# cxy1997/3D_adapt_auto_driving

Measured on AMD Instinct MI355X. Metric: KITTI scenes/s end-to-end eval_rcnn (joint RPN+RCNN, synthetic 16384-pt scenes), higher is better.
Workload: dtype f32; 1 GPU; BASELINE.json configs[2]: full PointRCNN RPN+RCNN inference, default.yaml shapes, random-init weights, batch=8 synthetic KITTI scenes x 16384 pts per GPU per step; scene=synth.scenes (SURVEY 8d: uniform clutter + ground + 10 dense cars), parallelism=scene-sharded x1, one final all_gather of detections, detections_gathered=652455, batch_slots=14, look_ahead=12, steps_per_launch=2

## Files before the change

### 3d_adapt_auto_driving_amd/csrc/mfma_stream.hpp

```cpp
#pragma once

#define RT_VM_DRAIN __builtin_amdgcn_s_waitcnt(0x0F70);
#define RT_LOAD_W(dst, rs, krow)                                                                          \
    _Pragma("unroll") for (int s = 0; s < 64; ++s)                                                        \
        dst[s] = __uint_as_float(__builtin_amdgcn_raw_buffer_load_b32(rs, lane_off, (unsigned int)((krow) + s) * 512u, 0)); \
    __builtin_amdgcn_sched_barrier(0);
#define RT_STAGE_HOOK_LO(T, wf, wn, RS, krow, FIRST, HOOK, LOFF)                                                     \
    {                                                                                                     \
        f32x4 a0 = *reinterpret_cast<const f32x4 *>((T) + j * RT_LD + 64 * h);                            \
        f32x4 a1 = *reinterpret_cast<const f32x4 *>((T) + (32 + j) * RT_LD + 64 * h);                     \
        _Pragma("unroll") for (int g = 0; g < 16; ++g) {                                                  \
            f32x4 n0 = a0, n1 = a1;                                                                       \
            if (g < 15) {                                                                                 \
                n0 = *reinterpret_cast<const f32x4 *>((T) + j * RT_LD + 64 * h + 4 * (g + 1));            \
                n1 = *reinterpret_cast<const f32x4 *>((T) + (32 + j) * RT_LD + 64 * h + 4 * (g + 1));     \
            }                                                                                             \
            __builtin_amdgcn_sched_barrier(0);                                                            \
            if ((FIRST) && g == 0) {                                                                      \
                const f32x16 zero = {0};                                                                  \
                acc0 = __builtin_amdgcn_mfma_f32_32x32x2f32(a0.x, wf[0], zero, 0, 0, 0);                  \
                acc1 = __builtin_amdgcn_mfma_f32_32x32x2f32(a1.x, wf[0], zero, 0, 0, 0);                  \
            } else {                                                                                      \
                acc0 = __builtin_amdgcn_mfma_f32_32x32x2f32(a0.x, wf[4 * g + 0], acc0, 0, 0, 0);          \
                acc1 = __builtin_amdgcn_mfma_f32_32x32x2f32(a1.x, wf[4 * g + 0], acc1, 0, 0, 0);          \
            }                                                                                             \
            _Pragma("unroll") for (int q = 0; q < 4; ++q)                                                 \
                wn[4 * g + q] = __uint_as_float(__builtin_amdgcn_raw_buffer_load_b32(                     \
                    RS, (LOFF), (unsigned int)((krow) + 4 * g + q) * 512u, 0));                           \
            __builtin_amdgcn_sched_barrier(0);                                                            \
            HOOK(g)                                                                                       \
            acc0 = __builtin_amdgcn_mfma_f32_32x32x2f32(a0.y, wf[4 * g + 1], acc0, 0, 0, 0);              \
            acc1 = __builtin_amdgcn_mfma_f32_32x32x2f32(a1.y, wf[4 * g + 1], acc1, 0, 0, 0);              \
            acc0 = __builtin_amdgcn_mfma_f32_32x32x2f32(a0.z, wf[4 * g + 2], acc0, 0, 0, 0);              \
            acc1 = __builtin_amdgcn_mfma_f32_32x32x2f32(a1.z, wf[4 * g + 2], acc1, 0, 0, 0);              \
            acc0 = __builtin_amdgcn_mfma_f32_32x32x2f32(a0.w, wf[4 * g + 3], acc0, 0, 0, 0);              \
            acc1 = __builtin_amdgcn_mfma_f32_32x32x2f32(a1.w, wf[4 * g + 3], acc1, 0, 0, 0);              \
            a0 = n0; a1 = n1;                                                                             \
        }                                                                                                 \
    }
#define RT_STAGE_HOOK(T, wf, wn, RS, krow, FIRST, HOOK) RT_STAGE_HOOK_LO(T, wf, wn, RS, krow, FIRST, HOOK, lane_off)
#define RT_NO_HOOK(g)
#define RT_STAGE(T, wf, wn, RS, krow, FIRST) RT_STAGE_HOOK(T, wf, wn, RS, krow, FIRST, RT_NO_HOOK)
#define RT_EPILOGUE(T, bias, RELU)                                                                        \
    {                                                                                                     \
        const float bcol = (bias);                                                                        \
        _Pragma("unroll") for (int r = 0; r < 16; ++r) {                                                  \
            const int row = (r & 3) + 8 * (r >> 2) + 4 * h;                                               \
            const float v0 = acc0[r] + bcol, v1 = acc1[r] + bcol;                                         \
            (T)[row * RT_LD + 32 * w + j] = (RELU) ? fmaxf(v0, 0.f) : v0;                                 \
            (T)[(32 + row) * RT_LD + 32 * w + j] = (RELU) ? fmaxf(v1, 0.f) : v1;                          \
        }                                                                                                 \
    }
```

### 3d_adapt_auto_driving_amd/csrc/rpn_tail.hip

```cpp
#include <hip/hip_runtime.h>

#include "common.hpp"
#include "mfma_stream.hpp"
#include "../../include/prcnn_hip.h"

namespace prcnn {

typedef float f32x16 __attribute__((ext_vector_type(16)));
typedef float f32x4 __attribute__((ext_vector_type(4)));

constexpr int RT_ROWS = 64;
constexpr int RT_LD = 128 + 4;
#ifndef RT_IROWS
#define RT_IROWS 4
#endif

struct RpnTailArgs {
    long rows;
    int n, m;
    const float *known;
    const int *idx;
    const float *weight;
    const float *wcat;
    const float *bcat;
    const float *wc2, *bc2;
    float *feats, *cls, *reg;
    int n_reg;
    unsigned int *ticket;
    int xcd_split;
    const float *xyz;
    float *boxes;
    float loc_scope, loc_bin_size, anchor[3];
};

__device__ __forceinline__ float fmod_two_pi(float a)
{
    constexpr double B0 = (double)(float)(2.0 * M_PI), B1 = B0 * 1099511627776.0 , B2 = B1 * 1099511627776.0;
    constexpr double I0 = 1.0 / B0, I1 = 1.0 / B1, I2 = 1.0 / B2;
    double r = __builtin_fabs((double)a);
    r = __builtin_fma(-__builtin_trunc(r * I2), B2, r);
    r = __builtin_fma(-__builtin_trunc(r * I1), B1, r);
    r = __builtin_fma(-__builtin_trunc(r * I0), B0, r);
    r = r < 0.0 ? r + B0 : r;
    r = r < 0.0 ? r + B0 : r;
    r = r >= B0 ? r - B0 : r;
    r = r >= B0 ? r - B0 : r;
    return __builtin_copysignf((float)r, a);
}

__global__ __launch_bounds__(256, 1) void rpn_tail_kernel(const RpnTailArgs a)
{
    __shared__ float T0[RT_ROWS * RT_LD];
    __shared__ float T1[RT_ROWS * RT_LD];
    __shared__ float X0[RT_ROWS * RT_LD];
    __shared__ float X1[RT_ROWS * RT_LD];
    __shared__ unsigned int slot[2];
    const int tid = threadIdx.x, lane = tid & 63, j = lane & 31, h = lane >> 5;
    const int w = __builtin_amdgcn_readfirstlane(tid >> 6);
    const int chunk = tid & 31, r0 = tid >> 5;
    const long tiles = (a.rows + RT_ROWS - 1) / RT_ROWS;
    const unsigned int lane_off = ((unsigned int)(64 * h) * 128u + (unsigned int)(32 * w + j)) * 4u;
    const __amdgpu_buffer_rsrc_t rs = __builtin_amdgcn_make_buffer_rsrc((void *)a.wcat, 0, 768 * 128 * 4, 0x00020000);
    const float wd0 = a.wc2[j], wd1 = a.wc2[j + 32], wd2 = a.wc2[j + 64], wd3 = a.wc2[j + 96], bd = a.bc2[0];
    const f32x4 *known4 = reinterpret_cast<const f32x4 *>(a.known);
    const float bias1 = a.bcat[32 * w + j], bias2 = a.bcat[128 + 32 * w + j], biasc = a.bcat[256 + 32 * w + j],
                biasr1 = a.bcat[384 + 32 * w + j], biasr2 = a.bcat[512 + 32 * w + j];

    int nx_i, nx_cloud;
    float nx_w;
#define RT_FETCH_IDX(tt)                                                                                  \
    {                                                                                                     \
        long ge = (tt) * RT_ROWS + 16 * w + lane / 3;                                                     \
        if (ge >= a.rows) ge = a.rows - 1;  \
        const long el = ge * 3 + lane % 3;                                                                \
        nx_i = lane < 48 ? a.idx[el] : 0;                                                                 \
        nx_w = lane < 48 ? a.weight[el] : 0.f;                                                            \
        nx_cloud = (int)(ge / a.n);                                                                       \
    }
    f32x4 f[RT_IROWS][3];
#define RT_INTERP_ISSUE(rr)                                                                               \
    _Pragma("unroll") for (int q = 0; q < RT_IROWS; ++q) {                                                \
        const long cloud = __builtin_amdgcn_readlane(nx_cloud, 3 * ((rr) + q));                           \
        _Pragma("unroll") for (int e = 0; e < 3; ++e) {                                                   \
            const int i = __builtin_amdgcn_readlane(nx_i, 3 * ((rr) + q) + e);                            \
            f[q][e] = known4[(cloud * a.m + i) * 64 + lane];                                              \
        }                                                                                                 \
    }
#define RT_INTERP_ROW(rr, q)                                                                              \
    {                                                                                                     \
        const float w0 = __builtin_bit_cast(float, __builtin_amdgcn_readlane(__builtin_bit_cast(int, nx_w), 3 * ((rr) + (q)))); \
        const float w1 = __builtin_bit_cast(float, __builtin_amdgcn_readlane(__builtin_bit_cast(int, nx_w), 3 * ((rr) + (q)) + 1)); \
        const float w2 = __builtin_bit_cast(float, __builtin_amdgcn_readlane(__builtin_bit_cast(int, nx_w), 3 * ((rr) + (q)) + 2)); \
        const f32x4 v = (w0 * f[q][0] + w1 * f[q][1]) + w2 * f[q][2];                                     \
        float *dst = (lane < 32 ? X0 : X1) + (16 * w + (rr) + (q)) * RT_LD + 4 * (lane & 31);             \
        *reinterpret_cast<f32x4 *>(dst) = v;                                                              \
    }
#define RT_SIDE(rr, g)                                                                                    \
    if ((g) == 2) { RT_INTERP_ISSUE(rr) }                                                                 \
    else if ((g) >= 10 && (g) < 10 + RT_IROWS) { RT_INTERP_ROW(rr, (g) - 10) }
#define RT_SIDE0(g) RT_SIDE(0, g)
#define RT_SIDE1(g) RT_SIDE(RT_IROWS, g)
#define RT_SIDE2(g) RT_SIDE(2 * RT_IROWS, g)
#define RT_SIDE3(g) RT_SIDE(3 * RT_IROWS, g)
    f32x4 co[4];
#define RT_ROWS_OUT(g, TT, T, dst, ld, live)                                                              \
    if ((g) == 1 || (g) == 4) {                                                                       \
        _Pragma("unroll") for (int i = 0; i < 4; ++i) co[i] = *reinterpret_cast<const f32x4 *>((T) + (r0 + 8 * (i + ((g) == 4 ? 4 : 0))) * RT_LD + 4 * chunk); \
    } else if ((g) == 3 || (g) == 6) {                                                                \
        _Pragma("unroll") for (int i = 0; i < 4; ++i) {                                               \
            const unsigned int gr = (unsigned int)(TT) * RT_ROWS + r0 + 8 * (i + ((g) == 6 ? 4 : 0)); \
            if ((live) && gr < (unsigned int)a.rows) *reinterpret_cast<f32x4 *>((dst) + (gr * (unsigned int)(ld) + 4u * chunk)) = co[i]; \
        }                                                                                             \
    }
    static_assert(RT_IROWS == 4, "four stages carry four rounds of four rows");

    if (tid == 0) { slot[0] = atomicAdd(a.ticket, 1u); }
    __syncthreads();
    long t = __builtin_amdgcn_readfirstlane((int)slot[0]);
    float wa[64], wb[64];
    f32x16 acc0, acc1;
    RT_LOAD_W(wa, rs, 0)
    if (t < tiles) {
        RT_FETCH_IDX(t)
#pragma unroll
        for (int rr = 0; rr < 16; rr += RT_IROWS) {
            RT_INTERP_ISSUE(rr)
#pragma unroll
            for (int q = 0; q < RT_IROWS; ++q) RT_INTERP_ROW(rr, q)
        }
    }
    long tp = 0;
    bool last = false;
    for (unsigned int served = 0; t < tiles; ++served) {
        if (tid == 0) slot[(served + 1) & 1] = atomicAdd(a.ticket, 1u);
        RT_VM_DRAIN
        lds_barrier();
#define RT_REG_OUT(g) RT_ROWS_OUT(g, tp, T1, a.reg, a.n_reg, served > 0 && 4 * chunk < a.n_reg)
        RT_STAGE_HOOK(X0, wa, wb, rs, 128, true, RT_REG_OUT)
        RT_VM_DRAIN
        RT_STAGE(X1, wb, wa, rs, 256, false)
        lds_barrier();
        const long tn = __builtin_amdgcn_readfirstlane((int)slot[(served + 1) & 1]);
        RT_FETCH_IDX(tn)
        RT_EPILOGUE(T0, bias1, true)
        lds_barrier();
        RT_VM_DRAIN
        RT_STAGE_HOOK(T0, wa, wb, rs, 384, true, RT_SIDE0)
        RT_EPILOGUE(T1, bias2, true)
        lds_barrier();
        RT_VM_DRAIN
#define RT_SIDE1F(g) RT_SIDE1(g) RT_ROWS_OUT(g, t, T1, a.feats, 128, true)
        RT_STAGE_HOOK(T1, wb, wa, rs, 512, true, RT_SIDE1F)
        RT_EPILOGUE(T0, biasc, true)
        lds_barrier();
        RT_VM_DRAIN
        float sd[8];
#define RT_SCORE(g)                                                                                       \
        if ((g) == 4) {                                                                                   \
            _Pragma("unroll") for (int p = 0; p < 8; ++p) {                                               \
                const float *ar = T0 + (r0 + 8 * p) * RT_LD + j;                                          \
                float v = fmaf(ar[0], wd0, 0.f);                                                          \
                v = fmaf(ar[32], wd1, v);                                                                 \
                v = fmaf(ar[64], wd2, v);                                                                 \
                sd[p] = fmaf(ar[96], wd3, v);                                                             \
            }                                                                                             \
        } else if ((g) >= 5 && (g) <= 9) {                                                                \
            float o[8];                                                                                   \
            _Pragma("unroll") for (int p = 0; p < 8; ++p) o[p] = __shfl_xor(sd[p], 16 >> ((g) - 5), 32);  \
            _Pragma("unroll") for (int p = 0; p < 8; ++p) sd[p] = __fadd_rn(sd[p], o[p]);                 \
        } else if ((g) == 14) {                                                                           \
            _Pragma("unroll") for (int p = 0; p < 8; ++p) {                                               \
                const unsigned int gr = (unsigned int)t * RT_ROWS + r0 + 8 * p;                           \
                if (j == 0 && gr < (unsigned int)a.rows) a.cls[gr] = __fadd_rn(sd[p], bd);                \
            }                                                                                             \
        }
#define RT_SIDE2S(g) RT_SIDE2(g) RT_SCORE(g)
        RT_STAGE_HOOK(T1, wa, wb, rs, 640, true, RT_SIDE2S)
        lds_barrier();
        RT_EPILOGUE(T0, biasr1, true)
        lds_barrier();
        RT_VM_DRAIN
        RT_STAGE_HOOK(T0, wb, wa, rs, 0, true, RT_SIDE3)
        RT_EPILOGUE(T1, biasr2, false)
        tp = t;
        t = tn;
        last = true;
    }
    if (last) {
        lds_barrier();
        if (4 * chunk < a.n_reg) {
#pragma unroll
            for (int i = 0; i < 8; ++i) {
                const int row = r0 + 8 * i;
                const unsigned int g = (unsigned int)tp * RT_ROWS + row;
                if (g < (unsigned int)a.rows)
                    *reinterpret_cast<f32x4 *>(a.reg + (g * (unsigned int)a.n_reg + 4u * chunk)) =
                        *reinterpret_cast<const f32x4 *>(T1 + row * RT_LD + 4 * chunk);
            }
        }
    }
    if (tid == 0) ticket_release(a.ticket);
}


constexpr int RD_NB = 12;
typedef float f32x4v __attribute__((ext_vector_type(4)));
template <bool DECODE, bool NARROW>
__global__ __launch_bounds__(256, 1) void rpn_tail_lin_kernel(const RpnTailArgs a)
{
    __shared__ float T0[RT_ROWS * RT_LD];
    __shared__ float T1[RT_ROWS * RT_LD];
    __shared__ float X0[RT_ROWS * RT_LD];
    __shared__ float X1[RT_ROWS * RT_LD];
    __shared__ unsigned int slot[2];
    const int tid = threadIdx.x, lane = tid & 63, j = lane & 31, h = lane >> 5;
    const int w = __builtin_amdgcn_readfirstlane(tid >> 6);
    const int chunk = tid & 31, r0 = tid >> 5;
    const long tiles = (a.rows + RT_ROWS - 1) / RT_ROWS;
    const unsigned int lane_off = ((unsigned int)(64 * h) * 128u + (unsigned int)(32 * w + j)) * 4u;
    const __amdgpu_buffer_rsrc_t rs = __builtin_amdgcn_make_buffer_rsrc((void *)a.wcat, 0, 512 * 128 * 4, 0x00020000);
    const float wd0 = a.wc2[j], wd1 = a.wc2[j + 32], wd2 = a.wc2[j + 64], wd3 = a.wc2[j + 96], bd = a.bc2[0];
    const f32x4 *known4 = reinterpret_cast<const f32x4 *>(a.known);
    const f32x4 bias1v = *reinterpret_cast<const f32x4 *>(a.bcat + 4 * j);
    const float bias2 = a.bcat[128 + 32 * w + j], biasc = a.bcat[256 + 32 * w + j], biasr1 = a.bcat[384 + 32 * w + j],
                biasr2 = a.bcat[512 + 32 * w + j];
    const int nrb = w & 1, ncb = w >> 1;
    const unsigned int lane_off_n = ((unsigned int)(64 * h) * 128u + (unsigned int)(32 * ncb + j)) * 4u;
    const unsigned int lane_off_x = ((unsigned int)(32 * (lane >> 4)) * 128u + (unsigned int)(64 + (lane & 15))) * 4u;
    const float biasn = a.bcat[512 + 32 * ncb + j], biasx = a.bcat[512 + 64 + (lane & 15)];
    int nx_i, nx_cloud;
    float nx_w;
    f32x4 fl[2][3];
#define RL_ISSUE(sl, s)                                                                                   \
    {                                                                                                     \
        const int q_ = 2 * (s) + h;                                                                       \
        const long cloud_ = __shfl(nx_cloud, 3 * q_);                                                     \
        _Pragma("unroll") for (int e = 0; e < 3; ++e) {                                                   \
            const int i_ = __shfl(nx_i, 3 * q_ + e);                                                      \
            fl[sl][e] = known4[(cloud_ * a.m + i_) * 32 + j];                                             \
        }                                                                                                 \
    }
#define RL_ROW(sl, s, XN)                                                                                 \
    {                                                                                                     \
        const int q_ = 2 * (s) + h;                                                                       \
        const float w0_ = __shfl(nx_w, 3 * q_), w1_ = __shfl(nx_w, 3 * q_ + 1), w2_ = __shfl(nx_w, 3 * q_ + 2); \
        f32x4 v_ = ((w0_ * fl[sl][0] + w1_ * fl[sl][1]) + w2_ * fl[sl][2]) + bias1v;                      \
        v_.x = fmaxf(v_.x, 0.f); v_.y = fmaxf(v_.y, 0.f); v_.z = fmaxf(v_.z, 0.f); v_.w = fmaxf(v_.w, 0.f); \
        *reinterpret_cast<f32x4 *>((XN) + (16 * w + q_) * RT_LD + 4 * j) = v_;                             \
    }
#define RL_SIDE(r, g, gi, gf)                                                                             \
    if ((g) == (gi)) { RL_ISSUE(0, 2 * (r)) RL_ISSUE(1, 2 * (r) + 1) }                                    \
    else if ((g) == (gf)) { RL_ROW(0, 2 * (r), Xn) }                                                      \
    else if ((g) == (gf) + 1) { RL_ROW(1, 2 * (r) + 1, Xn) }
    f32x4 co[4];
    const int dpart = lane & 3;
    const float *drow = T1 + (16 * w + (lane >> 2)) * RT_LD;
    const int dstart = dpart == 0 ? 0 : dpart == 1 ? RD_NB : dpart == 2 ? 4 * RD_NB + 1 : 6 * RD_NB + 4 - RD_NB;
    const int dexb = dpart == 0 ? 2 * RD_NB : dpart == 1 ? 3 * RD_NB : dpart == 2 ? 5 * RD_NB + 1 : 4 * RD_NB;
    const int dxo = dpart == 0 ? 0 : dpart == 1 ? 2 : dpart == 2 ? 0 : 1;
    const int dbo = dpart == 0 ? 0 : dpart == 1 ? 2 : dpart == 2 ? 6 : 1;
    float dv[RD_NB], dp = 0.f, dex = 0.f, dout = 0.f, dh = 0.f, dw = 0.f, dl = 0.f;
    int dbi = 0;
#define RL_DEC_READ(TT)                                                                                   \
    {                                                                                                     \
        _Pragma("unroll") for (int i = 0; i < RD_NB; ++i) dv[i] = drow[dstart + i];                        \
        unsigned int gr_ = (unsigned int)(TT) * RT_ROWS + 16 * w + (lane >> 2);                           \
        if (gr_ >= (unsigned int)a.rows) gr_ = (unsigned int)a.rows - 1u;                                  \
        dp = a.xyz[gr_ * 3u + dxo];                                                                        \
    }
#define RL_DEC_ARGMAX                                                                                     \
    {                                                                                                     \
        float bv_ = dv[0];                                                                                \
        dbi = 0;                                                                                          \
        _Pragma("unroll") for (int i = 1; i < RD_NB; ++i) {                                                \
            const bool tk_ = dv[i] > bv_ || (dv[i] != dv[i] && bv_ == bv_);                                \
            bv_ = tk_ ? dv[i] : bv_;                                                                      \
            dbi = tk_ ? i : dbi;                                                                          \
        }                                                                                                 \
        dex = drow[dexb + (dpart < 3 ? dbi : 0)];                                                          \
    }
#define RL_DEC_MATH                                                                                       \
    {                                                                                                     \
        const float fb_ = (float)dbi, bin_ = a.loc_bin_size;                                               \
        float loc_ = __fsub_rn(__fadd_rn(__fmul_rn(fb_, bin_), bin_ / 2), a.loc_scope);                    \
        loc_ = __fadd_rn(__fadd_rn(loc_, __fmul_rn(dex, bin_)), dp);                                       \
        const float apc_ = (float)((2.0 * M_PI) / RD_NB), apch_ = (float)(((2.0 * M_PI) / RD_NB) / 2.0);   \
        const float two_pi_ = (float)(2.0 * M_PI), pi_ = (float)M_PI;                                      \
        float ry_ = fmod_two_pi(__fadd_rn(__fmul_rn(fb_, apc_), __fmul_rn(dex, apch_)));           \
        ry_ = (ry_ != 0.f && ry_ < 0.f) ? __fadd_rn(ry_, two_pi_) : ry_;                                   \
        ry_ = ry_ > pi_ ? __fsub_rn(ry_, two_pi_) : ry_;                                                   \
        dh = __fadd_rn(__fmul_rn(dv[RD_NB - 3], a.anchor[0]), a.anchor[0]);                                \
        dw = __fadd_rn(__fmul_rn(dv[RD_NB - 2], a.anchor[1]), a.anchor[1]);                                \
        dl = __fadd_rn(__fmul_rn(dv[RD_NB - 1], a.anchor[2]), a.anchor[2]);                                \
        const float y_ = __fadd_rn(__fadd_rn(dp, dex), dh / 2);                                            \
        dout = dpart < 2 ? loc_ : dpart == 2 ? ry_ : y_;                                                   \
    }
#define RL_DEC_STORE(TT, live)                                                                            \
    {                                                                                                     \
        const unsigned int gr_ = (unsigned int)(TT) * RT_ROWS + 16 * w + (lane >> 2);                     \
        if ((live) && gr_ < (unsigned int)a.rows) {                                                        \
            float *o_ = a.boxes + gr_ * 7u;                                                                \
            o_[dbo] = dout;                                                                                \
            if (dpart == 3) { o_[3] = dh; o_[4] = dw; o_[5] = dl; }                                        \
        }                                                                                                 \
    }
#define RL_DECODE(g, TT, live)                                                                            \
    if ((g) == 1) RL_DEC_READ(TT)                                                                         \
    else if ((g) == 3) RL_DEC_ARGMAX                                                                      \
    else if ((g) == 5) RL_DEC_MATH                                                                        \
    else if ((g) == 7) RL_DEC_STORE(TT, live)

    XcdTickets tk;
    tk.rec = a.ticket; tk.tiles = (unsigned int)tiles; tk.dead = 0u;
    tk.chunk = a.xcd_split ? (unsigned int)((tiles + 7) / 8) : (unsigned int)tiles;
    tk.xcd = a.xcd_split ? (blockIdx.x & 7u) : 0u;
    if (tid == 0) { slot[0] = tk.issue(); }
    __syncthreads();
    long t = __builtin_amdgcn_readfirstlane((int)slot[0]);
    float wa[64], wb[64];
    f32x16 acc0, acc1;
    RT_LOAD_W(wa, rs, 0)
    if (t < tiles) {
        RT_FETCH_IDX(t)
        float *Xn = X0;
#pragma unroll
        for (int r = 0; r < 4; ++r) {
            RL_ISSUE(0, 2 * r) RL_ISSUE(1, 2 * r + 1)
            RL_ROW(0, 2 * r, Xn) RL_ROW(1, 2 * r + 1, Xn)
        }
    }
    long tp = 0;
    bool last = false;
    for (unsigned int served = 0; t < tiles; ++served) {
        if (tid == 0) slot[(served + 1) & 1] = tk.issue();
        RT_VM_DRAIN
        lds_barrier();
        const float *Xc = (served & 1) ? X1 : X0;
        float *Xn = (served & 1) ? X0 : X1;
        const long tn = __builtin_amdgcn_readfirstlane((int)slot[(served + 1) & 1]);
        RT_FETCH_IDX(tn)
#define RL_H1R(g) RT_ROWS_OUT(g, tp, T1, a.reg, a.n_reg, served > 0 && 4 * chunk < a.n_reg) RL_SIDE(0, g, 8, 13)
#define RL_H1D(g) RL_DECODE(g, tp, served > 0) RL_SIDE(0, g, 8, 13)
        if (DECODE) { RT_STAGE_HOOK(Xc, wa, wb, rs, 128, true, RL_H1D) }
        else { RT_STAGE_HOOK(Xc, wa, wb, rs, 128, true, RL_H1R) }
        lds_barrier();
        RT_EPILOGUE(T1, bias2, true)
        lds_barrier();
        RT_VM_DRAIN
#define RL_H2(g) RT_ROWS_OUT(g, t, T1, a.feats, 128, true) RL_SIDE(1, g, 2, 10)
        RT_STAGE_HOOK(T1, wb, wa, rs, 256, true, RL_H2)
        RT_EPILOGUE(T0, biasc, true)
        lds_barrier();
        RT_VM_DRAIN
        float sd[8];
#define RL_H3(g) RT_SCORE(g) RL_SIDE(2, g, 2, 10)
        RT_STAGE_HOOK_LO(T1, wa, wb, rs, 384, true, RL_H3, (NARROW ? lane_off_n : lane_off))
        lds_barrier();
        RT_EPILOGUE(T0, biasr1, true)
        lds_barrier();
        RT_VM_DRAIN
#define RL_H4(g) RL_SIDE(3, g, 2, 10)
        if (NARROW) {
            float wx[32];
            f32x4 accx;
            {
                const float *ap = T0 + (32 * nrb + j) * RT_LD + 64 * h;
                f32x4 a0 = *reinterpret_cast<const f32x4 *>(ap);
#pragma unroll
                for (int g = 0; g < 16; ++g) {
                    f32x4 n0 = a0;
                    if (g < 15) n0 = *reinterpret_cast<const f32x4 *>(ap + 4 * (g + 1));
                    __builtin_amdgcn_sched_barrier(0);
                    if (g == 0) {
                        const f32x16 zero = {0};
                        acc0 = __builtin_amdgcn_mfma_f32_32x32x2f32(a0.x, wb[0], zero, 0, 0, 0);
                    } else {
                        acc0 = __builtin_amdgcn_mfma_f32_32x32x2f32(a0.x, wb[4 * g + 0], acc0, 0, 0, 0);
                    }
#pragma unroll
                    for (int q = 0; q < 4; ++q)
                        wa[4 * g + q] = __uint_as_float(__builtin_amdgcn_raw_buffer_load_b32(rs, lane_off, (unsigned int)(4 * g + q) * 512u, 0));
#pragma unroll
                    for (int q = 0; q < 2; ++q)
                        wx[2 * g + q] = __uint_as_float(__builtin_amdgcn_raw_buffer_load_b32(rs, lane_off_x, (unsigned int)(384 + 2 * g + q) * 512u, 0));
                    __builtin_amdgcn_sched_barrier(0);
                    RL_H4(g)
                    acc0 = __builtin_amdgcn_mfma_f32_32x32x2f32(a0.y, wb[4 * g + 1], acc0, 0, 0, 0);
                    acc0 = __builtin_amdgcn_mfma_f32_32x32x2f32(a0.z, wb[4 * g + 2], acc0, 0, 0, 0);
                    acc0 = __builtin_amdgcn_mfma_f32_32x32x2f32(a0.w, wb[4 * g + 3], acc0, 0, 0, 0);
                    a0 = n0;
                }
                const float *xp = T0 + (16 * w + (lane & 15)) * RT_LD + 32 * (lane >> 4);
                f32x4 x = *reinterpret_cast<const f32x4 *>(xp);
#pragma unroll
                for (int q = 0; q < 8; ++q) {
                    f32x4 nx = x;
                    if (q < 7) nx = *reinterpret_cast<const f32x4 *>(xp + 4 * (q + 1));
                    if (q == 0) {
                        const f32x4v zero4 = {0.f, 0.f, 0.f, 0.f};
                        accx = __builtin_amdgcn_mfma_f32_16x16x4f32(x.x, wx[0], zero4, 0, 0, 0);
                    } else {
                        accx = __builtin_amdgcn_mfma_f32_16x16x4f32(x.x, wx[4 * q + 0], accx, 0, 0, 0);
                    }
                    accx = __builtin_amdgcn_mfma_f32_16x16x4f32(x.y, wx[4 * q + 1], accx, 0, 0, 0);
                    accx = __builtin_amdgcn_mfma_f32_16x16x4f32(x.z, wx[4 * q + 2], accx, 0, 0, 0);
                    accx = __builtin_amdgcn_mfma_f32_16x16x4f32(x.w, wx[4 * q + 3], accx, 0, 0, 0);
                    x = nx;
                }
            }
#pragma unroll
            for (int r = 0; r < 16; ++r) {
                const int row = 32 * nrb + (r & 3) + 8 * (r >> 2) + 4 * h;
                T1[row * RT_LD + 32 * ncb + j] = acc0[r] + biasn;
            }
#pragma unroll
            for (int r = 0; r < 4; ++r) T1[(16 * w + 4 * (lane >> 4) + r) * RT_LD + 64 + (lane & 15)] = accx[r] + biasx;
        } else {
            RT_STAGE_HOOK(T0, wb, wa, rs, 0, true, RL_H4)
            RT_EPILOGUE(T1, biasr2, false)
        }
        tp = t;
        t = tn;
        last = true;
    }
    if (last) {
        lds_barrier();
        if (DECODE) {
            RL_DEC_READ(tp) RL_DEC_ARGMAX RL_DEC_MATH RL_DEC_STORE(tp, true)
        } else if (4 * chunk < a.n_reg) {
#pragma unroll
            for (int i = 0; i < 8; ++i) {
                const int row = r0 + 8 * i;
                const unsigned int g = (unsigned int)tp * RT_ROWS + row;
                if (g < (unsigned int)a.rows)
                    *reinterpret_cast<f32x4 *>(a.reg + (g * (unsigned int)a.n_reg + 4u * chunk)) =
                        *reinterpret_cast<const f32x4 *>(T1 + row * RT_LD + 4 * chunk);
            }
        }
    }
    if (tid == 0) tk.release();
}

}

namespace prcnn {
unsigned int *next_ticket(hipStream_t st);

__global__ __launch_bounds__(256) void fmod_two_pi_selftest_kernel(long n, const float *__restrict__ a, float *__restrict__ mine,
                                                                   float *__restrict__ lib)
{
    const long i = (long)blockIdx.x * 256 + threadIdx.x;
    if (i >= n) return;
    mine[i] = fmod_two_pi(a[i]);
    lib[i] = fmodf(a[i], (float)(2.0 * M_PI));
}
}

using namespace prcnn;

extern "C" int prcnn_rpn_tail(int b, int n, int m, const float *known, const int *idx, const float *weight, const float *wcat,
                              const float *bcat, const float *wc2, const float *bc2, int n_reg, float *feats, float *cls,
                              float *reg, void *stream)
{
    PRCNN_REQUIRE(b >= 0 && n >= 0 && m >= 1 && n_reg >= 4 && n_reg <= 128 && n_reg % 4 == 0,
                  "rpn_tail: bad sizes (n_reg=%d must be a multiple of 4 in 4..128)", n_reg);
    const long rows = (long)b * n;
    if (rows == 0) return PRCNN_OK;
    PRCNN_REQUIRE(rows <= (1L << 23), "rpn_tail: too many points (32-bit element offsets)");
    PRCNN_REQUIRE(known && idx && weight && wcat && bcat && wc2 && bc2 && feats && cls && reg, "rpn_tail: null pointer");
    PRCNN_REQUIRE((((uintptr_t)known | (uintptr_t)feats | (uintptr_t)wcat | (uintptr_t)reg) & 15) == 0,
                  "rpn_tail: 16-byte alignment required");
    RpnTailArgs a;
    a.rows = rows; a.n = n; a.m = m; a.known = known; a.idx = idx; a.weight = weight;
    a.wcat = wcat; a.bcat = bcat; a.wc2 = wc2; a.bc2 = bc2; a.feats = feats; a.cls = cls; a.reg = reg; a.n_reg = n_reg;
    a.ticket = next_ticket((hipStream_t)stream);
    if (!a.ticket) { set_error("rpn_tail: cannot set up the tile ticket"); return PRCNN_ELAUNCH; }
    a.xcd_split = 0;
    const long tiles = (rows + RT_ROWS - 1) / RT_ROWS;
    const long cap = mfma_grid_cap() < 256 ? mfma_grid_cap() : 256;
    const long grid = tiles < cap ? tiles : cap;
    hipLaunchKernelGGL(rpn_tail_kernel, dim3((unsigned)grid), dim3(256), 0, (hipStream_t)stream, a);
    return check_launch("rpn_tail");
}


static int rpn_tail_lin_any(int b, int n, int m, const float *G, const int *idx, const float *weight, const float *wcat,
                            const float *bcat, const float *wc2, const float *bc2, int n_reg, float *feats, float *cls,
                            float *reg, const float *xyz, float *boxes, float loc_scope, float loc_bin_size, const float *anchor,
                            void *stream, const char *who)
{
    PRCNN_REQUIRE(b >= 0 && n >= 0 && m >= 1 && n_reg >= 4 && n_reg <= 128 && n_reg % 4 == 0,
                  "%s: bad sizes (n_reg=%d must be a multiple of 4 in 4..128)", who, n_reg);
    const long rows = (long)b * n;
    if (rows == 0) return PRCNN_OK;
    PRCNN_REQUIRE(rows <= (1L << 23), "%s: too many points (32-bit element offsets)", who);
    PRCNN_REQUIRE(G && idx && weight && wcat && bcat && wc2 && bc2 && feats && cls && (reg || boxes), "%s: null pointer", who);
    PRCNN_REQUIRE((((uintptr_t)G | (uintptr_t)feats | (uintptr_t)wcat | (uintptr_t)reg | (uintptr_t)bcat) & 15) == 0,
                  "%s: 16-byte alignment required", who);
    RpnTailArgs a;
    a.rows = rows; a.n = n; a.m = m; a.known = G; a.idx = idx; a.weight = weight;
    a.wcat = wcat; a.bcat = bcat; a.wc2 = wc2; a.bc2 = bc2; a.feats = feats; a.cls = cls; a.reg = reg; a.n_reg = n_reg;
    a.xyz = xyz; a.boxes = boxes; a.loc_scope = loc_scope; a.loc_bin_size = loc_bin_size;
    for (int i = 0; i < 3; ++i) a.anchor[i] = anchor ? anchor[i] : 0.f;
    a.ticket = next_ticket((hipStream_t)stream);
    if (!a.ticket) { set_error("%s: cannot set up the tile ticket", who); return PRCNN_ELAUNCH; }
    const int xcd_split = 1;
    const long tiles = (rows + RT_ROWS - 1) / RT_ROWS;
    static const long tail_cap = getenv("PRCNN_TAIL_GRID") && atol(getenv("PRCNN_TAIL_GRID")) > 0 ? atol(getenv("PRCNN_TAIL_GRID")) : 256;
    const long cap = mfma_grid_cap() < tail_cap ? mfma_grid_cap() : tail_cap;
    const long grid = tiles < cap ? tiles : cap;
    a.xcd_split = xcd_split && (grid >= 8 || grid == tiles);
    static const bool narrow_ok = !(getenv("PRCNN_TAIL_NARROW") && atoi(getenv("PRCNN_TAIL_NARROW")) == 0);
    const bool narrow = narrow_ok && n_reg > 64 && n_reg <= 80;
    if (boxes && narrow) hipLaunchKernelGGL((rpn_tail_lin_kernel<true, true>), dim3((unsigned)grid), dim3(256), 0, (hipStream_t)stream, a);
    else if (boxes) hipLaunchKernelGGL((rpn_tail_lin_kernel<true, false>), dim3((unsigned)grid), dim3(256), 0, (hipStream_t)stream, a);
    else if (narrow) hipLaunchKernelGGL((rpn_tail_lin_kernel<false, true>), dim3((unsigned)grid), dim3(256), 0, (hipStream_t)stream, a);
    else hipLaunchKernelGGL((rpn_tail_lin_kernel<false, false>), dim3((unsigned)grid), dim3(256), 0, (hipStream_t)stream, a);
    return check_launch(who);
}

extern "C" int prcnn_rpn_tail_lin(int b, int n, int m, const float *G, const int *idx, const float *weight, const float *wcat,
                                  const float *bcat, const float *wc2, const float *bc2, int n_reg, float *feats, float *cls,
                                  float *reg, void *stream)
{
    PRCNN_REQUIRE(reg || (long)b * n == 0, "rpn_tail_lin: null pointer");
    return rpn_tail_lin_any(b, n, m, G, idx, weight, wcat, bcat, wc2, bc2, n_reg, feats, cls, reg, nullptr, nullptr, 0.f, 0.f, nullptr,
                            stream, "rpn_tail_lin");
}

extern "C" int prcnn_selftest_fmod_two_pi(long n, const float *a, float *out_mine, float *out_lib, void *stream)
{
    PRCNN_REQUIRE(n >= 0, "selftest_fmod_two_pi: bad size");
    if (n == 0) return PRCNN_OK;
    PRCNN_REQUIRE(a && out_mine && out_lib, "selftest_fmod_two_pi: null pointer");
    hipLaunchKernelGGL(fmod_two_pi_selftest_kernel, dim3((unsigned)((n + 255) / 256)), dim3(256), 0, (hipStream_t)stream, n, a, out_mine, out_lib);
    return check_launch("selftest_fmod_two_pi");
}

extern "C" int prcnn_rpn_tail_boxes_supported(int channels, float loc_scope, float loc_bin_size, int num_head_bin, int xz_fine)
{
    return loc_bin_size > 0.f && (int)(loc_scope / loc_bin_size) * 2 == RD_NB && num_head_bin == RD_NB && xz_fine &&
           channels == 6 * RD_NB + 4;
}

extern "C" int prcnn_rpn_tail_lin_boxes(int b, int n, int m, const float *G, const int *idx, const float *weight, const float *wcat,
                                        const float *bcat, const float *wc2, const float *bc2, int n_reg, float loc_scope,
                                        float loc_bin_size, int num_head_bin, int xz_fine, const float *anchor_size_host,
                                        const float *xyz, float *feats, float *cls, float *boxes, void *stream)
{
    PRCNN_REQUIRE(prcnn_rpn_tail_boxes_supported(n_reg, loc_scope, loc_bin_size, num_head_bin, xz_fine),
                  "rpn_tail_lin_boxes: regression layout (%d channels, scope %g / bin %g, %d heading bins, xz_fine %d) not served",
                  n_reg, loc_scope, loc_bin_size, num_head_bin, xz_fine);
    PRCNN_REQUIRE(anchor_size_host && ((xyz && boxes) || (long)b * n == 0), "rpn_tail_lin_boxes: null pointer");
    return rpn_tail_lin_any(b, n, m, G, idx, weight, wcat, bcat, wc2, bc2, n_reg, feats, cls, nullptr, xyz, boxes, loc_scope, loc_bin_size,
                            anchor_size_host, stream, "rpn_tail_lin_boxes");
}
```

Measured before the change: 8876 scenes/s.

## Keep all four layer weight slices resident in registers instead of streaming per stage

Loads the weight slices for all four MLP stages of the RPN tail once per persistent block into separate register arrays, three of them pinned to AGPRs through inline asm constraints. The per-stage streaming buffer loads and the vector-memory drains between stages are removed, and a new stage macro runs MFMA without interleaved weight loads. This takes global weight traffic and waitcnt stalls off every tile. In exchange register use rises to about 290 floats per lane, which may lower occupancy or cause spills.

```diff
diff --git a/3d_adapt_auto_driving_amd/csrc/mfma_stream.hpp b/3d_adapt_auto_driving_amd/csrc/mfma_stream.hpp
--- a/3d_adapt_auto_driving_amd/csrc/mfma_stream.hpp
+++ b/3d_adapt_auto_driving_amd/csrc/mfma_stream.hpp
@@ -41,6 +41,40 @@
 #define RT_STAGE_HOOK(T, wf, wn, RS, krow, FIRST, HOOK) RT_STAGE_HOOK_LO(T, wf, wn, RS, krow, FIRST, HOOK, lane_off)
 #define RT_NO_HOOK(g)
 #define RT_STAGE(T, wf, wn, RS, krow, FIRST) RT_STAGE_HOOK(T, wf, wn, RS, krow, FIRST, RT_NO_HOOK)
+#define RT_LOAD_W_LO(dst, rs, krow, cnt, LOFF)                                                            \
+    _Pragma("unroll") for (int s = 0; s < (cnt); ++s)                                                     \
+        dst[s] = __uint_as_float(__builtin_amdgcn_raw_buffer_load_b32(rs, (LOFF), (unsigned int)((krow) + s) * 512u, 0));
+#define RT_PIN_AGPR(arr, cnt) _Pragma("unroll") for (int s = 0; s < (cnt); ++s) asm volatile("" : "+a"(arr[s]));
+#define RT_STAGE_RES(T, wf, FIRST, HOOK)                                                                  \
+    {                                                                                                     \
+        f32x4 a0 = *reinterpret_cast<const f32x4 *>((T) + j * RT_LD + 64 * h);                            \
+        f32x4 a1 = *reinterpret_cast<const f32x4 *>((T) + (32 + j) * RT_LD + 64 * h);                     \
+        _Pragma("unroll") for (int g = 0; g < 16; ++g) {                                                  \
+            f32x4 n0 = a0, n1 = a1;                                                                       \
+            if (g < 15) {                                                                                 \
+                n0 = *reinterpret_cast<const f32x4 *>((T) + j * RT_LD + 64 * h + 4 * (g + 1));            \
+                n1 = *reinterpret_cast<const f32x4 *>((T) + (32 + j) * RT_LD + 64 * h + 4 * (g + 1));     \
+            }                                                                                             \
+            __builtin_amdgcn_sched_barrier(0);                                                            \
+            if ((FIRST) && g == 0) {                                                                      \
+                const f32x16 zero = {0};                                                                  \
+                acc0 = __builtin_amdgcn_mfma_f32_32x32x2f32(a0.x, wf[0], zero, 0, 0, 0);                  \
+                acc1 = __builtin_amdgcn_mfma_f32_32x32x2f32(a1.x, wf[0], zero, 0, 0, 0);                  \
+            } else {                                                                                      \
+                acc0 = __builtin_amdgcn_mfma_f32_32x32x2f32(a0.x, wf[4 * g + 0], acc0, 0, 0, 0);          \
+                acc1 = __builtin_amdgcn_mfma_f32_32x32x2f32(a1.x, wf[4 * g + 0], acc1, 0, 0, 0);          \
+            }                                                                                             \
+            __builtin_amdgcn_sched_barrier(0);                                                            \
+            HOOK(g)                                                                                       \
+            acc0 = __builtin_amdgcn_mfma_f32_32x32x2f32(a0.y, wf[4 * g + 1], acc0, 0, 0, 0);              \
+            acc1 = __builtin_amdgcn_mfma_f32_32x32x2f32(a1.y, wf[4 * g + 1], acc1, 0, 0, 0);              \
+            acc0 = __builtin_amdgcn_mfma_f32_32x32x2f32(a0.z, wf[4 * g + 2], acc0, 0, 0, 0);              \
+            acc1 = __builtin_amdgcn_mfma_f32_32x32x2f32(a1.z, wf[4 * g + 2], acc1, 0, 0, 0);              \
+            acc0 = __builtin_amdgcn_mfma_f32_32x32x2f32(a0.w, wf[4 * g + 3], acc0, 0, 0, 0);              \
+            acc1 = __builtin_amdgcn_mfma_f32_32x32x2f32(a1.w, wf[4 * g + 3], acc1, 0, 0, 0);              \
+            a0 = n0; a1 = n1;                                                                             \
+        }                                                                                                 \
+    }
 #define RT_EPILOGUE(T, bias, RELU)                                                                        \
     {                                                                                                     \
         const float bcol = (bias);                                                                        \
diff --git a/3d_adapt_auto_driving_amd/csrc/rpn_tail.hip b/3d_adapt_auto_driving_amd/csrc/rpn_tail.hip
--- a/3d_adapt_auto_driving_amd/csrc/rpn_tail.hip
+++ b/3d_adapt_auto_driving_amd/csrc/rpn_tail.hip
@@ -317,9 +317,15 @@
     if (tid == 0) { slot[0] = tk.issue(); }
     __syncthreads();
     long t = __builtin_amdgcn_readfirstlane((int)slot[0]);
-    float wa[64], wb[64];
+    float wf2[64], wc1[64], wr1[64], wr2[64], wx[NARROW ? 32 : 1];
     f32x16 acc0, acc1;
-    RT_LOAD_W(wa, rs, 0)
+    RT_LOAD_W_LO(wf2, rs, 0, 64, lane_off)
+    RT_LOAD_W_LO(wc1, rs, 128, 64, lane_off)
+    RT_LOAD_W_LO(wr1, rs, 256, 64, lane_off)
+    RT_LOAD_W_LO(wr2, rs, 384, 64, (NARROW ? lane_off_n : lane_off))
+    if (NARROW) { RT_LOAD_W_LO(wx, rs, 384, 32, lane_off_x) }
+    RT_PIN_AGPR(wf2, 64) RT_PIN_AGPR(wc1, 64) RT_PIN_AGPR(wr1, 64)
+    __builtin_amdgcn_sched_barrier(0);
     if (t < tiles) {
         RT_FETCH_IDX(t)
         float *Xn = X0;
@@ -333,7 +339,6 @@
     bool last = false;
     for (unsigned int served = 0; t < tiles; ++served) {
         if (tid == 0) slot[(served + 1) & 1] = tk.issue();
-        RT_VM_DRAIN
         lds_barrier();
         const float *Xc = (served & 1) ? X1 : X0;
         float *Xn = (served & 1) ? X0 : X1;
@@ -341,27 +346,23 @@
         RT_FETCH_IDX(tn)
 #define RL_H1R(g) RT_ROWS_OUT(g, tp, T1, a.reg, a.n_reg, served > 0 && 4 * chunk < a.n_reg) RL_SIDE(0, g, 8, 13)
 #define RL_H1D(g) RL_DECODE(g, tp, served > 0) RL_SIDE(0, g, 8, 13)
-        if (DECODE) { RT_STAGE_HOOK(Xc, wa, wb, rs, 128, true, RL_H1D) }
-        else { RT_STAGE_HOOK(Xc, wa, wb, rs, 128, true, RL_H1R) }
+        if (DECODE) { RT_STAGE_RES(Xc, wf2, true, RL_H1D) }
+        else { RT_STAGE_RES(Xc, wf2, true, RL_H1R) }
         lds_barrier();
         RT_EPILOGUE(T1, bias2, true)
         lds_barrier();
-        RT_VM_DRAIN
 #define RL_H2(g) RT_ROWS_OUT(g, t, T1, a.feats, 128, true) RL_SIDE(1, g, 2, 10)
-        RT_STAGE_HOOK(T1, wb, wa, rs, 256, true, RL_H2)
+        RT_STAGE_RES(T1, wc1, true, RL_H2)
         RT_EPILOGUE(T0, biasc, true)
         lds_barrier();
-        RT_VM_DRAIN
         float sd[8];
 #define RL_H3(g) RT_SCORE(g) RL_SIDE(2, g, 2, 10)
-        RT_STAGE_HOOK_LO(T1, wa, wb, rs, 384, true, RL_H3, (NARROW ? lane_off_n : lane_off))
+        RT_STAGE_RES(T1, wr1, true, RL_H3)
         lds_barrier();
         RT_EPILOGUE(T0, biasr1, true)
         lds_barrier();
-        RT_VM_DRAIN
 #define RL_H4(g) RL_SIDE(3, g, 2, 10)
         if (NARROW) {
-            float wx[32];
             f32x4 accx;
             {
                 const float *ap = T0 + (32 * nrb + j) * RT_LD + 64 * h;
@@ -373,21 +374,15 @@
                     __builtin_amdgcn_sched_barrier(0);
                     if (g == 0) {
                         const f32x16 zero = {0};
-                        acc0 = __builtin_amdgcn_mfma_f32_32x32x2f32(a0.x, wb[0], zero, 0, 0, 0);
+                        acc0 = __builtin_amdgcn_mfma_f32_32x32x2f32(a0.x, wr2[0], zero, 0, 0, 0);
                     } else {
-                        acc0 = __builtin_amdgcn_mfma_f32_32x32x2f32(a0.x, wb[4 * g + 0], acc0, 0, 0, 0);
+                        acc0 = __builtin_amdgcn_mfma_f32_32x32x2f32(a0.x, wr2[4 * g + 0], acc0, 0, 0, 0);
                     }
-#pragma unroll
-                    for (int q = 0; q < 4; ++q)
-                        wa[4 * g + q] = __uint_as_float(__builtin_amdgcn_raw_buffer_load_b32(rs, lane_off, (unsigned int)(4 * g + q) * 512u, 0));
-#pragma unroll
-                    for (int q = 0; q < 2; ++q)
-                        wx[2 * g + q] = __uint_as_float(__builtin_amdgcn_raw_buffer_load_b32(rs, lane_off_x, (unsigned int)(384 + 2 * g + q) * 512u, 0));
                     __builtin_amdgcn_sched_barrier(0);
                     RL_H4(g)
-                    acc0 = __builtin_amdgcn_mfma_f32_32x32x2f32(a0.y, wb[4 * g + 1], acc0, 0, 0, 0);
-                    acc0 = __builtin_amdgcn_mfma_f32_32x32x2f32(a0.z, wb[4 * g + 2], acc0, 0, 0, 0);
-                    acc0 = __builtin_amdgcn_mfma_f32_32x32x2f32(a0.w, wb[4 * g + 3], acc0, 0, 0, 0);
+                    acc0 = __builtin_amdgcn_mfma_f32_32x32x2f32(a0.y, wr2[4 * g + 1], acc0, 0, 0, 0);
+                    acc0 = __builtin_amdgcn_mfma_f32_32x32x2f32(a0.z, wr2[4 * g + 2], acc0, 0, 0, 0);
+                    acc0 = __builtin_amdgcn_mfma_f32_32x32x2f32(a0.w, wr2[4 * g + 3], acc0, 0, 0, 0);
                     a0 = n0;
                 }
                 const float *xp = T0 + (16 * w + (lane & 15)) * RT_LD + 32 * (lane >> 4);
@@ -416,7 +411,7 @@
 #pragma unroll
             for (int r = 0; r < 4; ++r) T1[(16 * w + 4 * (lane >> 4) + r) * RT_LD + 64 + (lane & 15)] = accx[r] + biasx;
         } else {
-            RT_STAGE_HOOK(T0, wb, wa, rs, 0, true, RL_H4)
+            RT_STAGE_RES(T0, wr2, true, RL_H4)
             RT_EPILOGUE(T1, biasr2, false)
         }
         tp = t;
```

Measured after the change: 8748 scenes/s. 0.985x the previous value.
